# indrajeetadityaroy9/vit-inductive-bias-distillation

Hardware: AMD Instinct MI355X
Metric: distillation images/sec (BASD loss fwd+bwd+grad all-reduce), DeiT-S<-ResNet-50 @ bs256/GPU (higher is better)
Workload: dtype f32; 1 GPU; cfg2 DeiT-S<-ResNet-50 224x224; per_gpu_batch=256, global_batch=256, input_dtype=float32, layout=strided (CLS-sliced / channel-major views), backward=True, grad_allreduce_bytes=88202672, grad_allreduce=none at world size 1 (bucket packed, nothing to exchange), rank_readback=auto, readback_deferred_steps=1756, selector=basd_selector_chain mode 0, parallelism=dp1

## Files before the change

include/basd_hip.h:

```cpp
#ifndef BASD_HIP_H
#define BASD_HIP_H

#include <stdint.h>

#ifdef __cplusplus
extern "C" {
#endif

#ifndef __HIP_PLATFORM_AMD__
typedef struct ihipStream_t* hipStream_t;
#endif

#define BASD_OK 0
#define BASD_EINVAL (-1)
#define BASD_EUNSUPPORTED (-2)
#define BASD_DTYPE_F32 0
#define BASD_DTYPE_BF16 1
#define BASD_DTYPE_U8 2


int basd_gemm_nt(const void* a, int a_dtype, long a_sb, long a_sn, long a_sd, int a_rows_per_batch,
                 long a_batch_stride, const float* b, long ldb, long b_batch_stride, int M, int N, int K, int batch,
                 float* c, long ldc, long c_batch_stride, float scale, const float* bias, float beta,
                 float* colsum_part, float* col_mean, hipStream_t stream);
// ... 134 lines not shown
int basd_selector_chain_tail(const BasdSelectorChain* args, int kmax, int exact_k);
int basd_jacobi_lds_square_fits(int n);


int basd_token_weights(const void* const* attn_ptrs, int dtype, const float* mix, int L, long sb, long sh, long sq,
                       long sk, int B, int H, int A, int has_cls, int n_a, int n_t, int n_s, const int* atap0,
                       const int* atap1, const float* alam, const int* tap0, const int* tap1, const float* lam,
                       float* omega, float* omega_t, float* raw_out, hipStream_t stream);

int basd_student_project(const void* x, int dtype, long sb, long sn, int B, int n_s, int n_t, int D,
                         const float* omega, const int* tap0, const int* tap1, const float* lam, const int* range0,
                         const int* range1, float* mu, float* tr_s, float* a_prime, hipStream_t stream);

int basd_teacher_center(const void* const* tok_ptrs, int dtype, const float* mix, int L, long sb, long sn, long sd,
                        int B, int n, int D, const int* g0, const int* g1, const float* glam, const float* omega_t,
                        float* mu, float* tc, hipStream_t stream);
int basd_teacher_center_multi(const void* const* tok_ptrs, int dtype, const float* mix, int L, int G, long sb, long sn,
                              long sd, int B, int n, int D, const int* g0, const int* g1, const float* glam,
                              const float* omega_t, float* mu, float* tc, hipStream_t stream);
long basd_teacher_center_stream_scratch_floats(int G, int B, int n, int D);
int basd_teacher_center_stream(const void* const* tok_ptrs, int dtype, const float* mix, int L, int G, long sb, long sn,
                               long sd, int B, int n, int D, const int* g0, const int* g1, const float* glam,
                               const float* omega_t, float* mu, float* tc, float* scratch, hipStream_t stream);

int basd_gram_f64(const float* p, long p_batch_stride, int n, int D, int batch, double* g, long g_batch_stride,
                  hipStream_t stream);

int basd_gram_f64_split(const float* p, long p_batch_stride, int n, int D, int batch, int splits, double* slabs,
                        double* g, hipStream_t stream);

int basd_chol_f64(const double* g, long g_batch_stride, int n, int batch, double* l, long l_batch_stride,
                  hipStream_t stream);

int basd_stack_product(const double* la, const double* lb, long l_batch_stride, int n, int batch, int lb_period,
                       float* w, long w_batch_stride, hipStream_t stream);

int basd_procrustes_finalize(const float* w, long w_batch_stride, const float* sigma, int n, int n_s, int batch,
                             int t_period ,
                             const double* gb, long g_batch_stride, const float* omega, const int* tap0,
                             const int* tap1, const float* lam, const float* tr_s_part, int tr_slabs, float* tr_s,
                             float* tr_t, float* nuc, float* loss, float* k_prime, hipStream_t stream);

int basd_student_project_multi(const void* const* x_ptrs, int dtype, long sb, long sn, int E, int B, int n_s, int n_t,
                               int D, int ptrs_16B_aligned, const float* omega, long omega_e_stride, const int* tap0,
                               const int* tap1, const float* lam, const int* range0, const int* range1, float* mu,
                               float* tr_s, float* a_prime, hipStream_t stream);
int basd_student_grad_multi(const void* const* x_ptrs, int dtype, long sb, long sn, int E, int B, int n_s, int n_t,
                            int D, const float* omega, long omega_e_stride, const float* mu, const float* h,
                            const int* tap0, const int* tap1, const float* lam, const float* scale_ptr,
                            float scale_const, float* dx, const float* tnorm2, float* gomega, hipStream_t stream);
int basd_student_grad_fused(const void* const* x_ptrs, int dtype, long sb, long sn, int E, int B, int n_s, int n_t,
                            int D, int ptrs_16B_aligned, const float* omega, long omega_e_stride, const float* mu,
                            const float* k_prime, const float* a_prime, const int* tap0, const int* tap1,
                            const float* lam, const float* scale_ptr, float scale_const, float* dx,
                            hipStream_t stream);

typedef struct BasdProcrustesArgs {
    const void* const* student_ptrs;
    const void* const* student_host_ptrs;
    long s_dtype, s_sb, s_sn, s_aligned;
    const void* const* tok_ptrs;
    long t_dtype, t_sb, t_sn, t_sd;
    const void* const* attn_ptrs;
    long a_dtype, a_sb, a_sh, a_sq, a_sk;
    const float* mix;
    long E, L, G, B, n_s, n_t, d_s, d_t, H, A, has_cls, n_a, n, max_sweeps;
// ... 137 lines not shown
```

vit-inductive-bias-distillation_amd/basd_amd/_lib.py:

```python
from __future__ import annotations

import ctypes as C
import os
import threading

_HERE = os.path.dirname(os.path.abspath(__file__))
LIB_PATH = os.path.join(_HERE, "libbasd_hip.so")

vp, i32, i64, f32, f64 = C.c_void_p, C.c_int, C.c_long, C.c_float, C.c_double

SIGNATURES = {
    "basd_gemm_nt": [vp, i32, i64, i64, i64, i32, i64, vp, i64, i64, i32, i32, i32, i32, vp, i64, i64, f32, vp, f32,
                     vp, vp, vp],
    "basd_gemm_tn_splits": [i32],
    "basd_gemm_tn": [vp, vp, i32, i64, i64, i64, i64, i64, i64, i64, i64, i32, i32, i32, i32, i32, vp, vp, i32, vp,
                     vp, i64, i64, f32, vp],
    "basd_colmean_parts": [i32],
    "basd_colmean": [vp, i32, i64, i64, i64, i32, i64, i32, i32, i32, i32, vp, vp, vp],
    "basd_colmean_multi": [vp, i32, i64, i64, i64, i32, i32, i32, i32, i32, vp, vp, i32, vp],
    "basd_syrk_splits": [i32, i32, i32],
    "basd_syrk_multi": [vp, i32, i64, i64, i64, i32, i32, i32, i32, vp, vp, i32, vp, vp, i64, i32, vp, i32, i32, vp],
    "basd_jacobi_workspace_ints": [i32, i32],
    "basd_jacobi_twopass_workspace_bytes": [i32, i32, i32],
    "basd_jacobi_stacked_twopass": [vp, i64, i32, i32, vp, i32, i32, f32, vp, vp, vp],
# ... 6 lines not shown
    "basd_tridiag_workspace_bytes": [i32, i32],
    "basd_tridiag_tuning": [i32, i32, i32, i32, i32, i32],
    "basd_tridiag": [vp, i64, i32, i32, vp, vp, vp, vp, vp, vp],
    "basd_tridiag_ranked": [vp, i64, i32, i32, vp, vp, vp, vp, vp, i32, f64, i32, vp, vp, vp, vp],
    "basd_tridiag_ranked_gated": [vp, i64, i32, i32, vp, vp, vp, vp, vp, i32, f64, i32, vp, vp, vp, C.c_uint, i32, vp],
    "basd_flag_set": [vp, C.c_uint, vp],
    "basd_scale_unless_one": [vp, i64, vp, vp, vp],
    "basd_event_create": [vp],
    "basd_event_destroy": [vp],
    "basd_stream_wait_event": [vp, vp],
    "basd_tridiag_eigenvalues": [vp, vp, i32, i32, vp, vp],
    "basd_tridiag_apply_q": [vp, vp, i32, i32, i32, vp, vp, i32, i32, vp],
    "basd_tridiag_shifted_solve": [vp, vp, vp, i32, i32, i32, i32, vp, vp, vp],
    "basd_tridiag_mp_rank": [vp, vp, i32, i32, f64, i32, vp, vp, vp, vp, vp],
    "basd_tridiag_mp_rank_rank1": [vp, vp, vp, i32, i32, f64, f64, i32, vp, vp, vp, vp],
    "basd_tridiag_eigenvectors": [vp, vp, vp, vp, vp, i32, i32, i32, vp, vp, i32, vp],
    "basd_mp_rank": [vp, i32, i32, f64, i32, vp, vp, vp],
    "basd_grassmann_distance": [vp, i32, vp, vp, i32, vp, i32, vp, vp, vp],
    "basd_grassmann_distance_padded": [vp, i32, i32, vp, vp, i32, vp, i32, vp, vp],
    "basd_selector_tail": [vp] * 10 + [i32, i32, i32, i32] + [vp] * 14 + [vp],
    "basd_sqrt_clamp": [vp, vp, i64, vp],
    "basd_gram_finish": [vp, vp, i32, i32, i64, vp, vp, vp],
    "basd_cross_entropy": [vp, i32, i64, i32, i32, vp, vp, i64, f32, i64, vp, vp, vp],
    "basd_token_weights": [vp, i32, vp, i32, i64, i64, i64, i64, i32, i32, i32, i32, i32, i32, i32, vp, vp, vp, vp,
                           vp, vp, vp, vp, vp, vp],
    "basd_student_project": [vp, i32, i64, i64, i32, i32, i32, i32, vp, vp, vp, vp, vp, vp, vp, vp, vp, vp],
    "basd_teacher_center": [vp, i32, vp, i32, i64, i64, i64, i32, i32, i32, vp, vp, vp, vp, vp, vp, vp],
    "basd_teacher_center_multi": [vp, i32, vp, i32, i32, i64, i64, i64, i32, i32, i32, vp, vp, vp, vp, vp, vp, vp],
    "basd_teacher_center_stream_scratch_floats": [i32, i32, i32, i32],
    "basd_teacher_center_stream": [vp, i32, vp, i32, i32, i64, i64, i64, i32, i32, i32, vp, vp, vp, vp, vp, vp, vp, vp],
    "basd_gram_f64": [vp, i64, i32, i32, i32, vp, i64, vp],
    "basd_gram_f64_split": [vp, i64, i32, i32, i32, i32, vp, vp, vp],
    "basd_chol_f64": [vp, i64, i32, i32, vp, i64, vp],
    "basd_stack_product": [vp, vp, i64, i32, i32, i32, vp, i64, vp],
    "basd_procrustes_finalize": [vp, i64, vp, i32, i32, i32, i32, vp, i64, vp, vp, vp, vp, vp, i32, vp, vp, vp, vp,
                                 vp, vp],
    "basd_student_project_multi": [vp, i32, i64, i64, i32, i32, i32, i32, i32, i32, vp, i64, vp, vp, vp, vp, vp, vp,
                                   vp, vp, vp],
    "basd_student_grad_multi": [vp, i32, i64, i64, i32, i32, i32, i32, i32, vp, i64, vp, vp, vp, vp, vp, vp, f32, vp,
                                vp, vp, vp],
    "basd_student_grad_fused": [vp, i32, i64, i64, i32, i32, i32, i32, i32, i32, vp, i64, vp, vp, vp, vp, vp, vp, vp,
                                f32, vp, vp],
    "basd_procrustes_forward_fused": [vp, vp],
    "basd_procrustes_tuning": [i32],
    "basd_jacobi_plain4_fits": [i32],
    "basd_stack_product_t": [vp, vp, i64, i32, i32, i32, vp, i64, vp],
    "basd_kprime_from_transposed": [vp, i64, vp, i32, i32, vp, i64, i32, vp, i64, vp, vp],
    "basd_ustack_stash": [vp, i64, i32, i32, vp, i64, vp],
    "basd_ustack_from_transposed": [vp, i64, vp, i32, i32, vp, i64, vp, i64, vp, i32, vp, vp],
    "basd_resample_tokens": [vp, i32, i64, i64, i64, i32, i32, i32, i32, vp, vp, vp, vp, vp],
    "basd_resample_tokens_adjoint": [vp, i32, i32, i32, i32, vp, vp, vp, vp, vp, vp, vp],
    "basd_teacher_factor": [vp, i64, vp, i32, i32, i32, vp, vp, i64, vp, vp, vp, vp, vp, vp, vp, vp, vp],
    "basd_teacher_factor_tiled": [vp, i64, vp, i32, i32, i32, vp, vp, i64, vp, vp, vp, vp, vp, vp, vp, vp, vp, vp],
    "basd_mix_grad_tokens": [vp, vp, i32, i32, i64, i64, i64, i32, i32, i32, i32, vp, vp, vp, vp, vp],
    "basd_mix_grad_tokens_scratch_floats": [i32, i32, i32, i32],
    "basd_mix_grad_tokens_onepass": [vp, vp, i32, i32, i64, i64, i64, i32, i32, i32, i32, vp, vp, vp, vp, vp, vp],
    "basd_token_weight_bwd": [vp, vp, i32, i32, i32, i32, vp, vp, vp, vp, vp, vp, i32, i32, i64, i64, i64, i64, i32,
                              i32, i32, vp, vp, vp],
    "basd_build_angle_stack": [vp, i32, vp, i32, vp, vp],
    "basd_grassmann_distance_bwd": [vp, vp, i32, vp, vp, i32, vp, vp, i32, vp, vp],
    "basd_eigvec_k2": [vp, vp, i32, i32, i32, vp, vp],
    "basd_selector_chain": [vp],
    "basd_rank_certificate": [vp, vp, i32, i32, f64, vp, vp, vp],
    "basd_rank_certificate_scratch_bytes": [i32],
    "basd_debug_fill_lds": [C.c_uint, vp],
    "basd_selector_chain_tail": [vp, i32, i32],
# ... 107 lines not shown
```

vit-inductive-bias-distillation_amd/basd_amd/ops.py:

```python
from __future__ import annotations

from dataclasses import dataclass
from functools import lru_cache

import torch

from . import _lib

import os

F32, BF16 = 0, 1
MAX_SWEEPS = 20
TWO_PASS_SVD = True
TRANSPOSED_MIX_GRAD = True
TWO_PASS_LOG_LIMIT = 16 << 30
EIG_SOLVER = os.environ.get("BASD_EIG_SOLVER", "tridiag")
if os.environ.get("BASD_GEMM_SPLIT") in ("0", "1"):
    _lib.call("basd_gemm_tuning", int(os.environ["BASD_GEMM_SPLIT"]))
if os.environ.get("BASD_JACOBI_ORDERING") in ("0", "1"):
    _lib.call("basd_jacobi_ordering", int(os.environ["BASD_JACOBI_ORDERING"]))


def _stream() -> int:
    return torch._C._cuda_getCurrentRawStream(torch._C._cuda_getDevice())
# ... 475 lines not shown
    if any(o.stride() != out[0].stride() for o in out):
        out = [o.contiguous() for o in out]
    return out


class _ProcrustesPlan:

    def __init__(self, E, L, B, n_s, d_s, n_t, d_t, H, A, has_cls, need_bwd, need_mix_grad, want_sweeps, want_dx,
                 want_uw, dev):
        import ctypes
        self.E, self.L, self.B, self.n_s, self.d_s, self.n_t, self.d_t = E, L, B, n_s, d_s, n_t, d_t
        n_a = A - (1 if has_cls else 0)
        n = min(n_s, n_t)
        self.n, self.n_a = n, n_a
        self.tp = taps(n_t, n_s, dev) if n_t < n_s else None
        self.gt = taps(n_t, n_s, dev) if n_t > n_s else None
        self.atp = taps(n_a, n_s, dev)
        G = self.G = 1 if L == 1 else E
        f32 = dict(device=dev, dtype=torch.float32)
        slabs = (d_s + 31) // 32
        EB, GB = E * B, G * B
        self.need_bwd, self.need_mix_grad, self.want_dx, self.want_uw = need_bwd, need_mix_grad, want_dx, want_uw
        self.kept_sizes = [G * B * n_s, E * B * d_s, EB * n * d_s, EB * n * n if need_bwd else 0, 4 * EB,
                           (4 + 2 * E) if want_uw else 0]
        self.kept_padded = [(c + 63) // 64 * 64 for c in self.kept_sizes]
        self.kept_total = sum(self.kept_padded)
        g_splits = 1
        if GB < 1024 and d_t >= 512:
            g_splits = max(1, min(1024 // GB, d_t // 256, 16))
        self.g_splits = g_splits
        self.g_all = torch.empty((EB + GB + (g_splits * GB if g_splits > 1 else 0), n, n), device=dev, dtype=torch.float64)
        self.l_all = torch.empty((EB + GB, n, n), device=dev, dtype=torch.float64)
        self.W = torch.empty((EB, n, 2 * n), **f32)
        self.tc = torch.empty((G, B, n, d_t), **f32)
        sizes = [GB * n, GB * d_t, EB * slabs, EB * n]
        padded = [(c + 63) // 64 * 64 for c in sizes]
        self.omega_t, self.mu_t, self.tr_part, self.sigma = (
            piece[:c] for piece, c in zip(torch.split(torch.empty((sum(padded),), **f32), padded), sizes))
        self.ints = torch.empty((_lib.query("basd_jacobi_workspace_ints", EB, MAX_SWEEPS) + EB,), device=dev,
                                dtype=torch.int32)
        self.sweeps = self.ints[-EB:] if want_sweeps else None
        transposed_mix = bool(need_mix_grad and need_bwd and _lib.query("basd_jacobi_plain4_fits", n)
                              and (EB >= 128 or TRANSPOSED_MIX_GRAD == "force") and TRANSPOSED_MIX_GRAD)
        jac_bytes = _lib.query("basd_jacobi_twopass_workspace_bytes", n, EB, MAX_SWEEPS) \
            if TWO_PASS_SVD and not transposed_mix else 0
        if jac_bytes > TWO_PASS_LOG_LIMIT or (jac_bytes > (256 << 20)
                                              and jac_bytes > torch.cuda.mem_get_info(dev)[0] // 2):
            jac_bytes = 0
        self.jac_ws = torch.empty((jac_bytes // 8 + 1,), device=dev, dtype=torch.int64) if jac_bytes > 0 else None
        self.h = torch.empty((E, B, n, d_s), **f32) if want_dx else None
        self.w_stack = None
        self.sigma_u = None
        if transposed_mix:
            self.w_stack = torch.empty((EB, n, 2 * n), **f32)
            self.sigma_u = torch.empty((EB, n), **f32)
        self.host_ptrs = (ctypes.c_void_p * E)()

        a = self.args = _lib.ProcrustesArgs()
        a.student_host_ptrs = ctypes.cast(self.host_ptrs, ctypes.c_void_p)
        (a.E, a.L, a.G, a.B, a.n_s, a.n_t, a.d_s, a.d_t, a.H, a.A, a.has_cls, a.n_a, a.n, a.max_sweeps) = \
            E, L, G, B, n_s, n_t, d_s, d_t, H, A, int(has_cls), n_a, n, MAX_SWEEPS
        if self.atp:
            a.atap0, a.atap1, a.alam = self.atp.tap0.data_ptr(), self.atp.tap1.data_ptr(), self.atp.lam.data_ptr()
        if self.tp:
            a.tap0, a.tap1, a.lam = self.tp.tap0.data_ptr(), self.tp.tap1.data_ptr(), self.tp.lam.data_ptr()
            a.range0, a.range1 = self.tp.range0.data_ptr(), self.tp.range1.data_ptr()
        if self.gt:
            a.g0, a.g1, a.glam = self.gt.tap0.data_ptr(), self.gt.tap1.data_ptr(), self.gt.lam.data_ptr()
        a.omega_t, a.mu_t, a.tc, a.tr_part = (self.omega_t.data_ptr(), self.mu_t.data_ptr(), self.tc.data_ptr(),
                                              self.tr_part.data_ptr())
        a.g_all, a.l_all, a.W = self.g_all.data_ptr(), self.l_all.data_ptr(), self.W.data_ptr()
        a.sigma, a.jflags, a.sweeps = self.sigma.data_ptr(), self.ints.data_ptr(), _ptr(self.sweeps)
        a.h = _ptr(self.h)
        a.g_slabs = self.g_all[EB + GB:].data_ptr() if g_splits > 1 else None
        a.g_splits = g_splits
        a.jac_ws = _ptr(self.jac_ws)
        a.w_stack = _ptr(self.w_stack)
        a.sigma_u = _ptr(self.sigma_u)


_PROCRUSTES_PLANS: dict = {}


def procrustes_forward(students: list[torch.Tensor], teachers: list[torch.Tensor], attns: list[torch.Tensor],
                       mix: torch.Tensor, has_cls: bool, *, need_backward: bool = True,
                       want_sweeps: bool = False, need_mix_grad: bool = False,
                       grad_layers: torch.Tensor | None = None,
                       uwso_ce: torch.Tensor | None = None) -> ProcrustesContext:
    import ctypes
    E, L = len(students), len(teachers)
    students = [as_supported(s) for s in students]
    students = _check_common_layout([s if s.stride(2) == 1 else s.contiguous() for s in students],
                                    "student token tensors")
    teachers = _check_common_layout([as_supported(t) for t in teachers], "teacher token tensors")
    attns = _check_common_layout([as_supported(a) for a in attns], "teacher attention tensors")
    _require_cuda(*students, *teachers, *attns, mix)
    s0, t0, a0 = students[0], teachers[0], attns[0]
    dev = s0.device
    B, n_s, d_s = s0.shape
    _, n_t, d_t = t0.shape
    H, A = a0.shape[1], a0.shape[2]
    need_bwd = need_backward or grad_layers is not None
# ... 190 lines not shown
```

vit-inductive-bias-distillation_amd/csrc/fused.hip:

```cpp
#include "basd_common.h"
#include "../../include/basd_hip.h"

namespace basd {

__global__ void __launch_bounds__(256) uwso_combine_kernel(const float* __restrict__ ce, const float* __restrict__ loss_b,
                                                           int E, int B, float* __restrict__ out) {
    constexpr int CH = 32;
    __shared__ double red[CH][4];
    const int tid = threadIdx.x;
    double geo_sum = 0.;
    for (int e0 = 0; e0 < E; e0 += CH) {
        const int ne = E - e0 < CH ? E - e0 : CH;
        for (int e = 0; e < ne; ++e) {
            double acc = 0.;
            for (int b = tid; b < B; b += 256) acc += (double)loss_b[(long)(e0 + e) * B + b];
            for (int m = 32; m > 0; m >>= 1) acc += __shfl_xor(acc, m, 64);
            if ((tid & 63) == 0) red[e][tid >> 6] = acc;
        }
        __syncthreads();
        if (tid == 0)
            for (int e = 0; e < ne; ++e) {
                const float layer = (float)(((red[e][0] + red[e][1]) + (red[e][2] + red[e][3])) / (double)B);
                out[4 + E + e0 + e] = layer;
                geo_sum += (double)layer;
// ... 62 lines not shown
        BASD_TRY(basd_student_grad_multi(a->student_ptrs, (int)a->s_dtype, a->s_sb, a->s_sn, E, B, n_s, n, d_s, a->omega,
                                         om_stride, a->mu_s, a->h, a->tap0, a->tap1, a->lam, grad_layers,
                                         2.0f / (float)B, a->dx, nullptr, nullptr, st));
    }
#undef BASD_TRY
    return BASD_OK;
}

static int g_transposed_cores = 1;
int basd_procrustes_tuning(int transposed_cores) {
    if (transposed_cores >= 0) g_transposed_cores = transposed_cores > 2 ? 2 : transposed_cores;
    return BASD_OK;
}

int basd_procrustes_forward_fused(const BasdProcrustesArgs* a, hipStream_t st) {
    BASD_CHECK_ARG(a && a->student_ptrs && a->tok_ptrs && a->attn_ptrs && a->mix);
    const int E = (int)a->E, L = (int)a->L, G = (int)a->G, B = (int)a->B, n_s = (int)a->n_s, n_t = (int)a->n_t;
    const int d_s = (int)a->d_s, d_t = (int)a->d_t, H = (int)a->H, A = (int)a->A, n_a = (int)a->n_a, n = (int)a->n;
    const float* grad_layers_in = a->grad_layers;
    BASD_CHECK_ARG(E > 0 && L > 0 && (G == 1 || G == E) && B > 0 && n == (n_s < n_t ? n_s : n_t));
    int rc;
#define BASD_TRY(call)            \
    do {                          \
        rc = (call);              \
        if (rc != BASD_OK) return rc; \
    } while (0)
    int centred = BASD_EUNSUPPORTED;
    for (int g = 0; g < G; ++g) {
        BASD_TRY(basd_token_weights(a->attn_ptrs, (int)a->a_dtype, a->mix + (long)g * L, L, a->a_sb, a->a_sh, a->a_sq,
                                    a->a_sk, B, H, A, (int)a->has_cls, n_a, n, n_s, a->atap0, a->atap1, a->alam,
                                    a->tap0, a->tap1, a->lam, a->omega + (long)g * B * n_s,
                                    a->omega_t + (long)g * B * n, a->raw ? a->raw + (long)g * B * n_a : nullptr, st));
    }
    if (G > 1 && L >= 4 && basd_teacher_center_stream_scratch_floats(G, B, n, d_t) <= (long)E * B * 2 * n * n) {
        centred = basd_teacher_center_stream(a->tok_ptrs, (int)a->t_dtype, a->mix, L, G, a->t_sb, a->t_sn, a->t_sd, B, n,
                                             d_t, a->g0, a->g1, a->glam, a->omega_t, a->mu_t, a->tc, a->W, st);
        if (centred != BASD_OK && centred != BASD_EUNSUPPORTED) return centred;
    }
    if (G > 1 && centred != BASD_OK) {
        centred = basd_teacher_center_multi(a->tok_ptrs, (int)a->t_dtype, a->mix, L, G, a->t_sb, a->t_sn, a->t_sd, B, n,
                                            d_t, a->g0, a->g1, a->glam, a->omega_t, a->mu_t, a->tc, st);
        if (centred != BASD_OK && centred != BASD_EUNSUPPORTED) return centred;
    }
    for (int g = 0; g < G && centred != BASD_OK; ++g) {
        BASD_TRY(basd_teacher_center(a->tok_ptrs, (int)a->t_dtype, a->mix + (long)g * L, L, a->t_sb, a->t_sn, a->t_sd,
                                     B, n, d_t, a->g0, a->g1, a->glam, a->omega_t + (long)g * B * n,
                                     a->mu_t + (long)g * B * d_t, a->tc + (long)g * B * n * d_t, st));
    }
    const long om_stride = G == 1 ? 0 : (long)B * n_s;
    int slabs = (d_s + 31) / 32;
    rc = basd_student_project_multi(a->student_ptrs, (int)a->s_dtype, a->s_sb, a->s_sn, E, B, n_s, n, d_s,
                                    (int)a->s_aligned, a->omega, om_stride, a->tap0, a->tap1, a->lam, a->range0,
                                    a->range1, a->mu_s, a->tr_part, a->a_prime, st);
    if (rc == BASD_EUNSUPPORTED) {
        slabs = (d_s + 63) / 64;
        for (int e = 0; e < E; ++e)
            BASD_TRY(basd_student_project(a->student_host_ptrs[e], (int)a->s_dtype, a->s_sb, a->s_sn, B, n_s, n, d_s,
                                          a->omega + e * om_stride, a->tap0, a->tap1, a->lam, a->range0, a->range1,
                                          a->mu_s + (long)e * B * d_s, a->tr_part + (long)e * B * slabs,
                                          a->a_prime + (long)e * B * n * d_s, st));
    } else if (rc != BASD_OK) {
        return rc;
    }
    const long nn = (long)n * n;
    const int EB = E * B, GB = G * B;
    BASD_TRY(basd_gram_f64(a->a_prime, (long)n * d_s, n, d_s, EB, a->g_all, nn, st));
    if (a->g_slabs && a->g_splits > 1)
        BASD_TRY(basd_gram_f64_split(a->tc, (long)n * d_t, n, d_t, GB, (int)a->g_splits, a->g_slabs,
                                     a->g_all + (long)EB * nn, st));
    else
        BASD_TRY(basd_gram_f64(a->tc, (long)n * d_t, n, d_t, GB, a->g_all + (long)EB * nn, nn, st));
    BASD_TRY(basd_chol_f64(a->g_all, nn, n, EB + GB, a->l_all, nn, st));
    if ((a->raw == nullptr || a->w_stack != nullptr) && EB <= 65535 && basd_jacobi_plain4_fits(n) &&
        (g_transposed_cores == 2 || (g_transposed_cores == 1 && EB >= 128))) {
        BASD_TRY(basd_stack_product_t(a->l_all, a->l_all + (long)EB * nn, nn, n, EB, GB, a->W, 2 * nn, st));
        if (a->raw != nullptr) BASD_TRY(basd_ustack_stash(a->W, 2 * nn, n, EB, a->w_stack, 2 * nn, st));
        BASD_TRY(basd_jacobi_onesided(a->W, 2 * nn, n, n, n, EB, nullptr, a->sigma, n, (int)a->max_sweeps, 0.f,
                                      a->jflags, a->sweeps, st));
        BASD_TRY(basd_procrustes_finalize(a->W, 2 * nn, a->sigma, n, n_s, EB, GB, a->g_all + (long)EB * nn, nn, a->omega,
                                          a->tap0, a->tap1, a->lam, a->tr_part, slabs, a->tr_s, a->tr_t, a->nuc,
                                          a->loss_b, nullptr, st));
        if (a->k_prime)
            BASD_TRY(basd_kprime_from_transposed(a->W, 2 * nn, a->sigma, n, EB, a->l_all + (long)EB * nn, nn, GB,
                                                 a->W + nn, 2 * nn, a->k_prime, st));
        if (a->raw != nullptr) {
            BASD_CHECK_ARG(a->sigma_u != nullptr);
            BASD_TRY(basd_ustack_from_transposed(a->W, 2 * nn, a->sigma, n, EB, a->w_stack, 2 * nn, a->W + nn, 2 * nn,
                                                 a->sigma_u, (int)a->max_sweeps, a->jflags, st));
        }
        return procrustes_tail(a, grad_layers_in, E, B, n_s, n, d_s, EB, nn, om_stride, st);
    }
    BASD_TRY(basd_stack_product(a->l_all, a->l_all + (long)EB * nn, nn, n, EB, GB, a->W, 2 * nn, st));
    rc = BASD_EUNSUPPORTED;
    if (a->jac_ws)
        rc = basd_jacobi_stacked_twopass(a->W, 2 * nn, n, EB, a->sigma, n, (int)a->max_sweeps, 0.f, a->jac_ws, a->sweeps,
                                         st);
    if (rc == BASD_EUNSUPPORTED)
        rc = basd_jacobi_onesided(a->W, 2 * nn, n, 2 * n, n, EB, nullptr, a->sigma, n, (int)a->max_sweeps, 0.f,
                                  a->jflags, a->sweeps, st);
    if (rc != BASD_OK) return rc;
    BASD_TRY(basd_procrustes_finalize(a->W, 2 * nn, a->sigma, n, n_s, EB, GB, a->g_all + (long)EB * nn, nn, a->omega,
                                      a->tap0, a->tap1, a->lam, a->tr_part, slabs, a->tr_s, a->tr_t, a->nuc,
                                      a->loss_b, a->k_prime, st));
// ... 22 lines not shown
```

vit-inductive-bias-distillation_amd/csrc/procrustes.hip:

```cpp
#include "basd_common.h"
#include "../../include/basd_hip.h"

namespace basd {

typedef double f64x4 __attribute__((ext_vector_type(4)));

template <typename T>
__global__ void __launch_bounds__(256) token_weights_kernel(const void* const* __restrict__ attn_ptrs,
                                                            const float* __restrict__ mix, int L, long sb, long sh,
                                                            long sq, long sk, int H, int A, int has_cls, int n_a,
                                                            int n_t, int n_s, const int* __restrict__ atap0,
                                                            const int* __restrict__ atap1,
                                                            const float* __restrict__ alam,
                                                            const int* __restrict__ tap0,
                                                            const int* __restrict__ tap1,
                                                            const float* __restrict__ lam, float* __restrict__ omega,
                                                            float* __restrict__ omega_t, float* __restrict__ raw_out) {
    extern __shared__ float sm[];
    float* raw = sm;
    float* w = sm + n_a;
    __shared__ float red[32];
    const int b = blockIdx.x, tid = threadIdx.x;
    for (int j = tid; j < n_a; j += blockDim.x) {
        float acc = 0.f;
// ... 531 lines not shown
                Gb[(long)col * n + row] = acc[t][r];
            }
        }
    }
}

__global__ void __launch_bounds__(256) gram_f64_reduce_kernel(const double* __restrict__ slabs, long split_stride,
                                                              int splits, long count, double* __restrict__ G) {
    const long i = (long)blockIdx.x * 256 + threadIdx.x;
    if (i >= count) return;
    double acc = 0.;
    for (int s2 = 0; s2 < splits; ++s2) acc += slabs[(long)s2 * split_stride + i];
    G[i] = acc;
}

static bool gram_f64_shape(int n, int* waves, int* chunks, size_t* lds) {
    const int nt = (n + 15) / 16, ntiles = nt * (nt + 1) / 2;
    int w = (ntiles + G64_TPW - 1) / G64_TPW;
    if (w < 4) w = ntiles < 4 ? ntiles : 4;
    int c = 1;
    if (w > 16) {
        c = (ntiles + 16 * G64_TPW - 1) / (16 * G64_TPW);
        w = 16;
    }
    *waves = w;
    *chunks = c;
    *lds = sizeof(float) * (size_t)nt * 16 * G64_LD;
    if (*lds > 156 * 1024) return false;
    if (*lds > 48 * 1024)
        (void)hipFuncSetAttribute((const void*)gram_f64_kernel, hipFuncAttributeMaxDynamicSharedMemorySize, 156 * 1024);
    return true;
}

__device__ __forceinline__ int pk(int i, int j, int n) { return j * n - (j * (j - 1)) / 2 + (i - j); }

__global__ void __launch_bounds__(1024) chol_f64_kernel(const double* __restrict__ G, long g_batch_stride, int n,
                                                        double* __restrict__ Lout, long l_batch_stride) {
    extern __shared__ __attribute__((aligned(16))) double a[];
    double* col = a + (size_t)n * (n + 1) / 2;
    __shared__ double sh_piv;
    __shared__ double red[32];
    const int m = blockIdx.x, tid = threadIdx.x, nthr = blockDim.x, lane = tid & 63, wave = tid >> 6, nw = nthr >> 6;
    const double* Gm = G + (long)m * g_batch_stride;
    double dmax = 0.;
    for (int j = wave; j < n; j += nw)
        for (int i = j + lane; i < n; i += 64) {
            const double v = Gm[(long)i * n + j];
            a[pk(i, j, n)] = v;
            if (i == j) dmax = fmax(dmax, v);
        }
    for (int s = 32; s > 0; s >>= 1) dmax = fmax(dmax, __shfl_xor(dmax, s, 64));
    if (lane == 0) red[wave] = dmax;
    __syncthreads();
    dmax = 0.;
    for (int i = 0; i < nw; ++i) dmax = fmax(dmax, red[i]);
    const double thr = dmax * (double)n * 1e-15;
    for (int j = 0; j < n; ++j) {
        if (tid == 0) {
            const double d = a[pk(j, j, n)];
            sh_piv = d > thr ? sqrt(d) : 0.;
        }
        __syncthreads();
        const double piv = sh_piv;
        const double inv = piv > 0. ? 1. / piv : 0.;
        for (int i = j + tid; i < n; i += nthr) {
            const double v = (i == j) ? piv : a[pk(i, j, n)] * inv;
// ... 956 lines not shown
    if (dtype == BASD_DTYPE_F32) LAUNCH_SGF_T(float);
    else if (dtype == BASD_DTYPE_BF16) LAUNCH_SGF_T(__hip_bfloat16);
    else return BASD_EINVAL;
#undef LAUNCH_SGF_T
#undef LAUNCH_SGF
    BASD_RETURN_LAST();
}

int basd_student_project_multi(const void* const* x_ptrs, int dtype, long sb, long sn, int E, int B, int n_s, int n_t,
                               int D, int ptrs_16B_aligned, const float* omega, long omega_e_stride, const int* tap0,
                               const int* tap1, const float* lam, const int* range0, const int* range1, float* mu,
                               float* tr_s, float* a_prime, hipStream_t stream) {
    BASD_CHECK_ARG(x_ptrs && omega && mu && tr_s && a_prime && E > 0 && B > 0 && n_s > 0 && n_t > 0 && D > 0);
    BASD_CHECK_ARG((n_t == n_s) == (tap0 == nullptr));
    BASD_CHECK_ARG(E <= 65535 && B <= 65535);
    const int esz = dtype == BASD_DTYPE_F32 ? 4 : 2;
    const size_t lds = sizeof(float) * ((size_t)n_s * SP_W + 5 * (size_t)n_s);
    const bool ok = ptrs_16B_aligned && D % 4 == 0 && (sb * esz) % 16 == 0 && (sn * esz) % 16 == 0 &&
                    (esz == 4 || D % 8 == 0) && lds <= 96 * 1024;
    if (!ok) return BASD_EUNSUPPORTED;
    const dim3 grid((D + SP_W - 1) / SP_W, B, E);
    if (dtype == BASD_DTYPE_F32) {
        (void)hipFuncSetAttribute((const void*)student_project_v4_kernel<float>, hipFuncAttributeMaxDynamicSharedMemorySize, (int)lds);
        student_project_v4_kernel<float><<<grid, 256, lds, stream>>>(x_ptrs, sb, sn, n_s, n_t, D, omega, omega_e_stride, tap0, tap1, lam, range0, range1, mu, tr_s, a_prime);
    } else if (dtype == BASD_DTYPE_BF16) {
        (void)hipFuncSetAttribute((const void*)student_project_v4_kernel<__hip_bfloat16>, hipFuncAttributeMaxDynamicSharedMemorySize, (int)lds);
        student_project_v4_kernel<__hip_bfloat16><<<grid, 256, lds, stream>>>(x_ptrs, sb, sn, n_s, n_t, D, omega, omega_e_stride, tap0, tap1, lam, range0, range1, mu, tr_s, a_prime);
    } else {
        return BASD_EINVAL;
    }
    BASD_RETURN_LAST();
}

int basd_resample_tokens(const void* x, int dtype, long sb, long sn, long sd, int B, int n_in, int n_out, int D,
                         const int* tap0, const int* tap1, const float* lam, float* out, hipStream_t stream) {
    BASD_CHECK_ARG(x && tap0 && tap1 && lam && out && B > 0 && n_in > 0 && n_out > 0 && D > 0);
    const dim3 grid(n_out, B);
    if (dtype == BASD_DTYPE_F32)
        resample_tokens_kernel<float><<<grid, 128, 0, stream>>>((const float*)x, sb, sn, sd, n_in, n_out, D, tap0, tap1, lam, out);
    else if (dtype == BASD_DTYPE_BF16)
        resample_tokens_kernel<__hip_bfloat16><<<grid, 128, 0, stream>>>((const __hip_bfloat16*)x, sb, sn, sd, n_in, n_out, D, tap0, tap1, lam, out);
    else
        return BASD_EINVAL;
    BASD_RETURN_LAST();
}

int basd_resample_tokens_adjoint(const float* dy, int B, int n_in, int n_out, int D, const int* tap0,
                                 const int* tap1, const float* lam, const int* range0, const int* range1, float* dx,
                                 hipStream_t stream) {
    BASD_CHECK_ARG(dy && tap0 && tap1 && lam && range0 && range1 && dx && B > 0 && n_in > 0 && n_out > 0 && D > 0);
    resample_tokens_adjoint_kernel<<<dim3(n_in, B), 128, 0, stream>>>(dy, n_in, n_out, D, tap0, tap1, lam, range0, range1, dx);
    BASD_RETURN_LAST();
}

}
```

Baseline: 165,100 images/s.

## Fuse Gram f64 accumulation into teacher centering and student projection kernels

Adds two kernels that compute the f64 Gram matrix with MFMA inside the teacher-centering and student-projection passes, working on LDS tiles as they are produced. This removes the separate basd_gram_f64 launches and their re-read of the centred teacher tensor and projected student activations. When no mix gradient is needed, the teacher's centred tensor is no longer allocated or written. In exchange the student kernel now runs one block per (batch, E) instead of splitting D across blocks, which lowers parallelism, and LDS use goes up.

After: 156,500 images/s. 0.948x the previous value.

```diff
diff --git a/include/basd_hip.h b/include/basd_hip.h
--- a/include/basd_hip.h
+++ b/include/basd_hip.h
@@ -190,6 +190,17 @@
 int basd_chol_f64(const double* g, long g_batch_stride, int n, int batch, double* l, long l_batch_stride,
                   hipStream_t stream);
 
+int basd_teacher_center_gram_fits(int n, int gathered);
+int basd_teacher_center_gram(const void* const* tok_ptrs, int dtype, const float* mix, int L, long sb, long sn, long sd,
+                             int B, int n, int D, const int* g0, const int* g1, const float* glam,
+                             const float* omega_t, float* mu, float* tc, int splits, double* slabs, double* g,
+                             hipStream_t stream);
+int basd_student_project_gram_multi(const void* const* x_ptrs, int dtype, long sb, long sn, int E, int B, int n_s,
+                                    int n_t, int D, int ptrs_16B_aligned, const float* omega, long omega_e_stride,
+                                    const int* tap0, const int* tap1, const float* lam, const int* range0,
+                                    const int* range1, float* mu, float* tr_s, float* a_prime, double* g,
+                                    long g_batch_stride, hipStream_t stream);
+
 int basd_stack_product(const double* la, const double* lb, long l_batch_stride, int n, int batch, int lb_period,
                        float* w, long w_batch_stride, hipStream_t stream);
 
diff --git a/vit-inductive-bias-distillation_amd/basd_amd/_lib.py b/vit-inductive-bias-distillation_amd/basd_amd/_lib.py
--- a/vit-inductive-bias-distillation_amd/basd_amd/_lib.py
+++ b/vit-inductive-bias-distillation_amd/basd_amd/_lib.py
@@ -62,6 +62,11 @@
     "basd_gram_f64": [vp, i64, i32, i32, i32, vp, i64, vp],
     "basd_gram_f64_split": [vp, i64, i32, i32, i32, i32, vp, vp, vp],
     "basd_chol_f64": [vp, i64, i32, i32, vp, i64, vp],
+    "basd_teacher_center_gram_fits": [i32, i32],
+    "basd_teacher_center_gram": [vp, i32, vp, i32, i64, i64, i64, i32, i32, i32, vp, vp, vp, vp, vp, vp, i32, vp, vp,
+                                 vp],
+    "basd_student_project_gram_multi": [vp, i32, i64, i64, i32, i32, i32, i32, i32, i32, vp, i64, vp, vp, vp, vp, vp,
+                                        vp, vp, vp, vp, i64, vp],
     "basd_stack_product": [vp, vp, i64, i32, i32, i32, vp, i64, vp],
     "basd_procrustes_finalize": [vp, i64, vp, i32, i32, i32, i32, vp, i64, vp, vp, vp, vp, vp, i32, vp, vp, vp, vp,
                                  vp, vp],
diff --git a/vit-inductive-bias-distillation_amd/basd_amd/ops.py b/vit-inductive-bias-distillation_amd/basd_amd/ops.py
--- a/vit-inductive-bias-distillation_amd/basd_amd/ops.py
+++ b/vit-inductive-bias-distillation_amd/basd_amd/ops.py
@@ -531,7 +531,8 @@
         self.g_all = torch.empty((EB + GB + (g_splits * GB if g_splits > 1 else 0), n, n), device=dev, dtype=torch.float64)
         self.l_all = torch.empty((EB + GB, n, n), device=dev, dtype=torch.float64)
         self.W = torch.empty((EB, n, 2 * n), **f32)
-        self.tc = torch.empty((G, B, n, d_t), **f32)
+        fused_teacher = G == 1 and bool(_lib.query("basd_teacher_center_gram_fits", n, int(bool(self.gt))))
+        self.tc = torch.empty((G, B, n, d_t), **f32) if need_mix_grad or not fused_teacher else None
         sizes = [GB * n, GB * d_t, EB * slabs, EB * n]
         padded = [(c + 63) // 64 * 64 for c in sizes]
         self.omega_t, self.mu_t, self.tr_part, self.sigma = (
@@ -566,7 +567,7 @@
             a.range0, a.range1 = self.tp.range0.data_ptr(), self.tp.range1.data_ptr()
         if self.gt:
             a.g0, a.g1, a.glam = self.gt.tap0.data_ptr(), self.gt.tap1.data_ptr(), self.gt.lam.data_ptr()
-        a.omega_t, a.mu_t, a.tc, a.tr_part = (self.omega_t.data_ptr(), self.mu_t.data_ptr(), self.tc.data_ptr(),
+        a.omega_t, a.mu_t, a.tc, a.tr_part = (self.omega_t.data_ptr(), self.mu_t.data_ptr(), _ptr(self.tc),
                                               self.tr_part.data_ptr())
         a.g_all, a.l_all, a.W = self.g_all.data_ptr(), self.l_all.data_ptr(), self.W.data_ptr()
         a.sigma, a.jflags, a.sweeps = self.sigma.data_ptr(), self.ints.data_ptr(), _ptr(self.sweeps)
diff --git a/vit-inductive-bias-distillation_amd/csrc/fused.hip b/vit-inductive-bias-distillation_amd/csrc/fused.hip
--- a/vit-inductive-bias-distillation_amd/csrc/fused.hip
+++ b/vit-inductive-bias-distillation_amd/csrc/fused.hip
@@ -118,6 +118,18 @@
                                     a->tap0, a->tap1, a->lam, a->omega + (long)g * B * n_s,
                                     a->omega_t + (long)g * B * n, a->raw ? a->raw + (long)g * B * n_a : nullptr, st));
     }
+    const long nn = (long)n * n;
+    const int EB = E * B, GB = G * B;
+    const int t_splits = a->g_slabs && a->g_splits > 1 ? (int)a->g_splits : 1;
+    bool t_gram = false;
+    if (G == 1) {
+        centred = basd_teacher_center_gram(a->tok_ptrs, (int)a->t_dtype, a->mix, L, a->t_sb, a->t_sn, a->t_sd, B, n, d_t,
+                                           a->g0, a->g1, a->glam, a->omega_t, a->mu_t, a->tc, t_splits, a->g_slabs,
+                                           a->g_all + (long)EB * nn, st);
+        if (centred != BASD_OK && centred != BASD_EUNSUPPORTED) return centred;
+        t_gram = centred == BASD_OK;
+    }
+    BASD_CHECK_ARG(t_gram || a->tc != nullptr);
     if (G > 1 && L >= 4 && basd_teacher_center_stream_scratch_floats(G, B, n, d_t) <= (long)E * B * 2 * n * n) {
         centred = basd_teacher_center_stream(a->tok_ptrs, (int)a->t_dtype, a->mix, L, G, a->t_sb, a->t_sn, a->t_sd, B, n,
                                              d_t, a->g0, a->g1, a->glam, a->omega_t, a->mu_t, a->tc, a->W, st);
@@ -135,7 +147,12 @@
     }
     const long om_stride = G == 1 ? 0 : (long)B * n_s;
     int slabs = (d_s + 31) / 32;
-    rc = basd_student_project_multi(a->student_ptrs, (int)a->s_dtype, a->s_sb, a->s_sn, E, B, n_s, n, d_s,
+    rc = basd_student_project_gram_multi(a->student_ptrs, (int)a->s_dtype, a->s_sb, a->s_sn, E, B, n_s, n, d_s,
+                                         (int)a->s_aligned, a->omega, om_stride, a->tap0, a->tap1, a->lam, a->range0,
+                                         a->range1, a->mu_s, a->tr_part, a->a_prime, a->g_all, nn, st);
+    const bool s_gram = rc == BASD_OK;
+    if (rc == BASD_EUNSUPPORTED)
+        rc = basd_student_project_multi(a->student_ptrs, (int)a->s_dtype, a->s_sb, a->s_sn, E, B, n_s, n, d_s,
                                     (int)a->s_aligned, a->omega, om_stride, a->tap0, a->tap1, a->lam, a->range0,
                                     a->range1, a->mu_s, a->tr_part, a->a_prime, st);
     if (rc == BASD_EUNSUPPORTED) {
@@ -148,13 +165,11 @@
     } else if (rc != BASD_OK) {
         return rc;
     }
-    const long nn = (long)n * n;
-    const int EB = E * B, GB = G * B;
-    BASD_TRY(basd_gram_f64(a->a_prime, (long)n * d_s, n, d_s, EB, a->g_all, nn, st));
-    if (a->g_slabs && a->g_splits > 1)
-        BASD_TRY(basd_gram_f64_split(a->tc, (long)n * d_t, n, d_t, GB, (int)a->g_splits, a->g_slabs,
+    if (!s_gram) BASD_TRY(basd_gram_f64(a->a_prime, (long)n * d_s, n, d_s, EB, a->g_all, nn, st));
+    if (!t_gram && t_splits > 1)
+        BASD_TRY(basd_gram_f64_split(a->tc, (long)n * d_t, n, d_t, GB, t_splits, a->g_slabs,
                                      a->g_all + (long)EB * nn, st));
-    else
+    else if (!t_gram)
         BASD_TRY(basd_gram_f64(a->tc, (long)n * d_t, n, d_t, GB, a->g_all + (long)EB * nn, nn, st));
     BASD_TRY(basd_chol_f64(a->g_all, nn, n, EB + GB, a->l_all, nn, st));
     if ((a->raw == nullptr || a->w_stack != nullptr) && EB <= 65535 && basd_jacobi_plain4_fits(n) &&
diff --git a/vit-inductive-bias-distillation_amd/csrc/procrustes.hip b/vit-inductive-bias-distillation_amd/csrc/procrustes.hip
--- a/vit-inductive-bias-distillation_amd/csrc/procrustes.hip
+++ b/vit-inductive-bias-distillation_amd/csrc/procrustes.hip
@@ -587,6 +587,296 @@
     return true;
 }
 
+constexpr int PG_TPW = 3, PG_ROWS = 64;
+
+__device__ __forceinline__ void pg_tiles_of_wave(int wave, int ntiles, int (&ti)[PG_TPW], int (&tj)[PG_TPW]) {
+#pragma unroll
+    for (int t = 0; t < PG_TPW; ++t) {
+        const int lin = wave + 4 * t;
+        int r = 0;
+        while ((r + 1) * (r + 2) / 2 <= lin) ++r;
+        ti[t] = lin < ntiles ? r : -1;
+        tj[t] = lin < ntiles ? lin - r * (r + 1) / 2 : -1;
+    }
+}
+
+__device__ __forceinline__ void pg_chunk_mfma(const float* tile, const int (&ti)[PG_TPW], const int (&tj)[PG_TPW],
+                                              int lane, f64x4 (&acc)[PG_TPW]) {
+    const int i16 = lane & 15, kq = lane >> 4;
+#pragma unroll 1
+    for (int g = 0; g < G64_BK / 16; ++g) {
+#pragma unroll
+        for (int t = 0; t < PG_TPW; ++t) {
+            if (ti[t] < 0) continue;
+            const float4 a = *(const float4*)(tile + (ti[t] * 16 + i16) * G64_LD + g * 16 + 4 * kq);
+            const float4 bb = *(const float4*)(tile + (tj[t] * 16 + i16) * G64_LD + g * 16 + 4 * kq);
+            acc[t] = __builtin_amdgcn_mfma_f64_16x16x4f64((double)a.x, (double)bb.x, acc[t], 0, 0, 0);
+            acc[t] = __builtin_amdgcn_mfma_f64_16x16x4f64((double)a.y, (double)bb.y, acc[t], 0, 0, 0);
+            acc[t] = __builtin_amdgcn_mfma_f64_16x16x4f64((double)a.z, (double)bb.z, acc[t], 0, 0, 0);
+            acc[t] = __builtin_amdgcn_mfma_f64_16x16x4f64((double)a.w, (double)bb.w, acc[t], 0, 0, 0);
+        }
+    }
+}
+
+__device__ __forceinline__ void pg_store(double* __restrict__ Gb, int n, const int (&ti)[PG_TPW],
+                                         const int (&tj)[PG_TPW], int lane, const f64x4 (&acc)[PG_TPW]) {
+#pragma unroll
+    for (int t = 0; t < PG_TPW; ++t) {
+        if (ti[t] < 0) continue;
+        const int col = tj[t] * 16 + (lane & 15);
+#pragma unroll
+        for (int r = 0; r < 4; ++r) {
+            const int row = ti[t] * 16 + (lane >> 4) + 4 * r;
+            if (row < n && col < n) {
+                Gb[(long)row * n + col] = acc[t][r];
+                Gb[(long)col * n + row] = acc[t][r];
+            }
+        }
+    }
+}
+
+template <typename T>
+__global__ void __launch_bounds__(256) teacher_center_gram_kernel(const void* const* __restrict__ tok_ptrs,
+                                                                  const float* __restrict__ mix, int L, long sb,
+                                                                  long sn, long sd, int n, int D,
+                                                                  const float* __restrict__ omega_t,
+                                                                  float* __restrict__ mu_out, float* __restrict__ Tc,
+                                                                  double* __restrict__ G, long g_split_stride) {
+    __shared__ __attribute__((aligned(16))) float raw[G64_BK * PG_ROWS];
+    __shared__ __attribute__((aligned(16))) float tile[PG_ROWS * G64_LD];
+    __shared__ __attribute__((aligned(16))) float mu[G64_BK];
+    __shared__ float wt[PG_ROWS];
+    const int s = blockIdx.x, S = gridDim.x, b = blockIdx.y, tid = threadIdx.x, lane = tid & 63, wave = tid >> 6;
+    const int nt = (n + 15) / 16, total = G64_BK * n;
+    const bool feat_fast = sd == 1;
+    bool vec = sb % 4 == 0 && (feat_fast ? sn % 4 == 0 : (sn == 1 && sd == n));
+    for (int l = 0; l < L; ++l) vec = vec && ((uintptr_t)tok_ptrs[l] & (4 * sizeof(T) - 1)) == 0;
+    const bool tc_vec = Tc != nullptr && D % 4 == 0 && ((uintptr_t)Tc & 15) == 0;
+    int ti[PG_TPW], tj[PG_TPW];
+    pg_tiles_of_wave(wave, nt * (nt + 1) / 2, ti, tj);
+    f64x4 acc[PG_TPW];
+#pragma unroll
+    for (int t = 0; t < PG_TPW; ++t) acc[t] = f64x4{0., 0., 0., 0.};
+    int j0[2], dd0[2], ddl[2];
+#pragma unroll
+    for (int h = 0; h < 2; ++h) {
+        const int e0 = 4 * (tid + 256 * h);
+        if (feat_fast) {
+            j0[h] = e0 >> 5;
+            dd0[h] = e0 & 31;
+            ddl[h] = dd0[h] + 3;
+        } else {
+            dd0[h] = e0 / n;
+            j0[h] = e0 - dd0[h] * n;
+            ddl[h] = (e0 + 3) / n;
+        }
+    }
+    const long base = (long)b * sb;
+    float4 pv[2];
+    auto fetch = [&](int k0) {
+#pragma unroll
+        for (int h = 0; h < 2; ++h) {
+            float x[4] = {0.f, 0.f, 0.f, 0.f};
+            if (4 * (tid + 256 * h) < total) {
+                if (vec && k0 + ddl[h] < D) {
+                    const long off = base + (long)(k0 + dd0[h]) * sd + (long)j0[h] * sn;
+                    for (int l = 0; l < L; ++l) {
+                        const float m = mix[l];
+                        const float4 t4 = ld4f((const BASD_GLOBAL_AS T*)tok_ptrs[l] + off);
+                        x[0] = fmaf(m, t4.x, x[0]); x[1] = fmaf(m, t4.y, x[1]);
+                        x[2] = fmaf(m, t4.z, x[2]); x[3] = fmaf(m, t4.w, x[3]);
+                    }
+                } else {
+                    int j = j0[h], dd = dd0[h];
+#pragma unroll
+                    for (int i = 0; i < 4; ++i) {
+                        if (k0 + dd < D) {
+                            const long off = base + (long)(k0 + dd) * sd + (long)j * sn;
+                            for (int l = 0; l < L; ++l)
+                                x[i] = fmaf(mix[l], ldg_f32((const BASD_GLOBAL_AS T*)tok_ptrs[l] + off), x[i]);
+                        }
+                        if (feat_fast) ++dd;
+                        else if (++j == n) { j = 0; ++dd; }
+                    }
+                }
+            }
+            pv[h] = make_float4(x[0], x[1], x[2], x[3]);
+        }
+    };
+    for (int j = tid; j < n; j += 256) wt[j] = omega_t[(long)b * n + j];
+    for (int i = tid; i < PG_ROWS * G64_LD; i += 256) tile[i] = 0.f;
+    int k0 = s * G64_BK;
+    if (k0 < D) fetch(k0);
+    for (; k0 < D; k0 += G64_BK * S) {
+#pragma unroll
+        for (int h = 0; h < 2; ++h) {
+            const int e0 = 4 * (tid + 256 * h);
+            if (e0 < total) *(float4*)(raw + e0) = pv[h];
+        }
+        if (k0 + G64_BK * S < D) fetch(k0 + G64_BK * S);
+        __syncthreads();
+        if (tid < G64_BK) {
+            float a = 0.f;
+            if (feat_fast) {
+#pragma unroll 8
+                for (int j = 0; j < n; ++j) a = fmaf(wt[j], raw[j * G64_BK + tid], a);
+            } else {
+#pragma unroll 8
+                for (int j = 0; j < n; ++j) a = fmaf(wt[j], raw[tid * n + j], a);
+            }
+            mu[tid] = a;
+            if (k0 + tid < D) mu_out[(long)b * D + k0 + tid] = a;
+        }
+        __syncthreads();
+        for (int idx = tid; idx < n * (G64_BK / 4); idx += 256) {
+            const int j = idx >> 3, c4 = (idx & 7) * 4;
+            float4 v;
+            if (feat_fast) {
+                v = *(const float4*)(raw + j * G64_BK + c4);
+            } else {
+                v.x = raw[c4 * n + j]; v.y = raw[(c4 + 1) * n + j];
+                v.z = raw[(c4 + 2) * n + j]; v.w = raw[(c4 + 3) * n + j];
+            }
+            const float4 m4 = *(const float4*)(mu + c4);
+            v.x -= m4.x; v.y -= m4.y; v.z -= m4.z; v.w -= m4.w;
+            *(float4*)(tile + j * G64_LD + c4) = v;
+            if (Tc) {
+                const int k = k0 + c4;
+                float* o = Tc + ((long)b * n + j) * D + k;
+                if (tc_vec && k + 3 < D) {
+                    *(float4*)o = v;
+                } else {
+                    if (k < D) o[0] = v.x;
+                    if (k + 1 < D) o[1] = v.y;
+                    if (k + 2 < D) o[2] = v.z;
+                    if (k + 3 < D) o[3] = v.w;
+                }
+            }
+        }
+        __syncthreads();
+        pg_chunk_mfma(tile, ti, tj, lane, acc);
+    }
+    pg_store(G + (long)s * g_split_stride + (long)b * n * n, n, ti, tj, lane, acc);
+}
+
+constexpr int SPG_NR = 7;
+template <typename T, bool PREFETCH>
+__global__ void __launch_bounds__(256, 4) student_project_gram_kernel(
+    const void* const* __restrict__ x_ptrs, long sb, long sn, int n_s, int n_t, int D,
+    const float* __restrict__ omega, long omega_e_stride, const int* __restrict__ tap0, const int* __restrict__ tap1,
+    const float* __restrict__ lam, const int* __restrict__ range0, const int* __restrict__ range1,
+    float* __restrict__ mu_out, float* __restrict__ tr_part, float* __restrict__ Ap, double* __restrict__ G,
+    long g_batch_stride) {
+    extern __shared__ __attribute__((aligned(16))) float sm[];
+    float* xs = sm;
+    float* w = sm + (long)n_s * SP_W;
+    float* c0 = w + n_s;
+    float* c1 = c0 + n_s;
+    int* t0 = (int*)(c1 + n_s);
+    int* t1 = t0 + n_s;
+    float* tile = sm + ((37 * n_s + 3) & ~3);
+    float (*red)[SP_W] = (float (*)[SP_W])tile;
+    __shared__ __attribute__((aligned(16))) float mu[SP_W];
+    __shared__ float scratch[32];
+    const int b = blockIdx.x, e = blockIdx.y, B = gridDim.x, tid = threadIdx.x, lane = tid & 63, wave = tid >> 6;
+    const int fq = tid & 7, rg = tid >> 3, c4 = 4 * fq;
+    const int slabs = (D + SP_W - 1) / SP_W, nt = (n_t + 15) / 16, rows_pad = nt * 16;
+    const BASD_GLOBAL_AS T* Xb = (const BASD_GLOBAL_AS T*)x_ptrs[e] + (long)b * sb;
+    const float* om = omega + (long)e * omega_e_stride + (long)b * n_s;
+    int ti[PG_TPW], tj[PG_TPW];
+    pg_tiles_of_wave(wave, nt * (nt + 1) / 2, ti, tj);
+    f64x4 gacc[PG_TPW];
+#pragma unroll
+    for (int t = 0; t < PG_TPW; ++t) gacc[t] = f64x4{0., 0., 0., 0.};
+    for (int n = tid; n < n_s; n += 256) {
+        const float wn = om[n];
+        w[n] = wn;
+        if (tap0) {
+            const float l1 = lam[n];
+            c0[n] = (1.f - l1) * wn;
+            c1[n] = l1 * wn;
+            t0[n] = tap0[n];
+            t1[n] = tap1[n];
+        }
+    }
+    float4 pv[SPG_NR];
+    auto fetch = [&](int d0) {
+        const bool lv = d0 + c4 < D;
+        const BASD_GLOBAL_AS T* p = Xb + d0 + (long)rg * sn + c4;
+#pragma unroll
+        for (int i = 0; i < SPG_NR; ++i, p += 32 * sn) {
+            pv[i] = make_float4(0.f, 0.f, 0.f, 0.f);
+            if (lv && rg + 32 * i < n_s) pv[i] = ld4f(p);
+        }
+    };
+    if (PREFETCH) fetch(0);
+    for (int sl = 0; sl < slabs; ++sl) {
+        const int d0 = sl * SP_W;
+        const bool live = d0 + c4 < D;
+        __syncthreads();
+        if (PREFETCH) {
+#pragma unroll
+            for (int i = 0; i < SPG_NR; ++i) {
+                const int n = rg + 32 * i;
+                if (n < n_s) *(float4*)(xs + n * SP_W + c4) = pv[i];
+            }
+            if (sl + 1 < slabs) fetch(d0 + SP_W);
+        } else {
+            for (int n = rg; n < n_s; n += 32) {
+                float4 v = make_float4(0.f, 0.f, 0.f, 0.f);
+                if (live) v = ld4f(Xb + d0 + (long)n * sn + c4);
+                *(float4*)(xs + n * SP_W + c4) = v;
+            }
+        }
+        __syncthreads();
+        float4 acc = make_float4(0.f, 0.f, 0.f, 0.f);
+        for (int n = rg; n < n_s; n += 32) {
+            const float4 v = *(const float4*)(xs + n * SP_W + c4);
+            const float wn = w[n];
+            acc.x = fmaf(wn, v.x, acc.x); acc.y = fmaf(wn, v.y, acc.y);
+            acc.z = fmaf(wn, v.z, acc.z); acc.w = fmaf(wn, v.w, acc.w);
+        }
+        *(float4*)(&red[rg][c4]) = acc;
+        __syncthreads();
+        if (tid < SP_W) {
+            float m = 0.f;
+#pragma unroll
+            for (int q = 0; q < 32; ++q) m += red[q][tid];
+            mu[tid] = m;
+            if (d0 + tid < D) mu_out[((long)e * B + b) * D + d0 + tid] = m;
+        }
+        __syncthreads();
+        const float4 m4 = *(const float4*)(mu + c4);
+        float part = 0.f;
+        if (live)
+            for (int n = rg; n < n_s; n += 32) {
+                const float4 v = *(const float4*)(xs + n * SP_W + c4);
+                const float cx = v.x - m4.x, cy = v.y - m4.y, cz = v.z - m4.z, cw = v.w - m4.w;
+                part = fmaf(w[n], fmaf(cx, cx, fmaf(cy, cy, fmaf(cz, cz, cw * cw))), part);
+            }
+        const float tr = block_sum(part, scratch);
+        if (tid == 0) tr_part[((long)e * B + b) * slabs + sl] = tr;
+        float* Ab = Ap + ((long)e * B + b) * n_t * D + d0 + c4;
+        for (int j = rg; j < rows_pad; j += 32) {
+            float4 a = make_float4(0.f, 0.f, 0.f, 0.f);
+            if (live && j < n_t) {
+                const int n0 = range0 ? range0[j] : j, n1 = range1 ? range1[j] : j + 1;
+                for (int n = n0; n < n1; ++n) {
+                    const float cw = tap0 ? (t0[n] == j ? c0[n] : 0.f) + (t1[n] == j ? c1[n] : 0.f) : w[n];
+                    const float4 v = *(const float4*)(xs + n * SP_W + c4);
+                    a.x = fmaf(cw, v.x - m4.x, a.x); a.y = fmaf(cw, v.y - m4.y, a.y);
+                    a.z = fmaf(cw, v.z - m4.z, a.z); a.w = fmaf(cw, v.w - m4.w, a.w);
+                }
+                *(float4*)(Ab + (long)j * D) = a;
+            }
+            *(float4*)(tile + j * G64_LD + c4) = a;
+        }
+        __syncthreads();
+        pg_chunk_mfma(tile, ti, tj, lane, gacc);
+    }
+    pg_store(G + ((long)e * B + b) * g_batch_stride, n_t, ti, tj, lane, gacc);
+}
+
 __device__ __forceinline__ int pk(int i, int j, int n) { return j * n - (j * (j - 1)) / 2 + (i - j); }
 
 __global__ void __launch_bounds__(1024) chol_f64_kernel(const double* __restrict__ G, long g_batch_stride, int n,
@@ -1609,6 +1899,66 @@
     BASD_RETURN_LAST();
 }
 
+int basd_teacher_center_gram_fits(int n, int gathered) { return n > 0 && n <= PG_ROWS && !gathered; }
+
+int basd_teacher_center_gram(const void* const* tok_ptrs, int dtype, const float* mix, int L, long sb, long sn, long sd,
+                             int B, int n, int D, const int* g0, const int* g1, const float* glam,
+                             const float* omega_t, float* mu, float* tc, int splits, double* slabs, double* g,
+                             hipStream_t stream) {
+    BASD_CHECK_ARG(tok_ptrs && mix && omega_t && mu && g && L > 0 && B > 0 && n > 0 && D > 0);
+    BASD_CHECK_ARG((g0 == nullptr) == (g1 == nullptr) && (g0 == nullptr) == (glam == nullptr));
+    BASD_CHECK_ARG(splits >= 1 && splits <= 64 && (splits == 1 || slabs != nullptr) && B <= 65535);
+    if (!basd_teacher_center_gram_fits(n, g0 != nullptr)) return BASD_EUNSUPPORTED;
+    const long count = (long)B * n * n;
+    double* out = splits > 1 ? slabs : g;
+    const dim3 grid(splits, B);
+    if (dtype == BASD_DTYPE_F32)
+        teacher_center_gram_kernel<float><<<grid, 256, 0, stream>>>(tok_ptrs, mix, L, sb, sn, sd, n, D, omega_t, mu, tc, out, count);
+    else if (dtype == BASD_DTYPE_BF16)
+        teacher_center_gram_kernel<__hip_bfloat16><<<grid, 256, 0, stream>>>(tok_ptrs, mix, L, sb, sn, sd, n, D, omega_t, mu, tc, out, count);
+    else
+        return BASD_EINVAL;
+    if (splits > 1)
+        gram_f64_reduce_kernel<<<(unsigned)((count + 255) / 256), 256, 0, stream>>>(slabs, count, splits, count, g);
+    BASD_RETURN_LAST();
+}
+
+int basd_student_project_gram_multi(const void* const* x_ptrs, int dtype, long sb, long sn, int E, int B, int n_s,
+                                    int n_t, int D, int ptrs_16B_aligned, const float* omega, long omega_e_stride,
+                                    const int* tap0, const int* tap1, const float* lam, const int* range0,
+                                    const int* range1, float* mu, float* tr_s, float* a_prime, double* g,
+                                    long g_batch_stride, hipStream_t stream) {
+    BASD_CHECK_ARG(x_ptrs && omega && mu && tr_s && a_prime && g && E > 0 && B > 0 && n_s > 0 && n_t > 0 && D > 0);
+    BASD_CHECK_ARG((n_t == n_s) == (tap0 == nullptr));
+    BASD_CHECK_ARG(E <= 65535 && B <= 65535 && ((uintptr_t)a_prime & 15) == 0);
+    if (n_t > PG_ROWS) return BASD_EUNSUPPORTED;
+    const int esz = dtype == BASD_DTYPE_F32 ? 4 : 2;
+    const int rows_pad = (n_t + 15) / 16 * 16, tile_floats = rows_pad * G64_LD > 32 * SP_W ? rows_pad * G64_LD : 32 * SP_W;
+    const size_t lds = sizeof(float) * ((size_t)((37 * n_s + 3) & ~3) + tile_floats);
+    const bool ok = ptrs_16B_aligned && D % 4 == 0 && (sb * esz) % 16 == 0 && (sn * esz) % 16 == 0 &&
+                    (esz == 4 || D % 8 == 0) && lds <= 96 * 1024;
+    if (!ok) return BASD_EUNSUPPORTED;
+    const dim3 grid(B, E);
+#define LAUNCH_SPG(TY, PF)                                                                                            \
+    do {                                                                                                              \
+        (void)hipFuncSetAttribute((const void*)student_project_gram_kernel<TY, PF>,                                   \
+                                  hipFuncAttributeMaxDynamicSharedMemorySize, (int)lds);                              \
+        student_project_gram_kernel<TY, PF><<<grid, 256, lds, stream>>>(x_ptrs, sb, sn, n_s, n_t, D, omega,            \
+                                                                        omega_e_stride, tap0, tap1, lam, range0,      \
+                                                                        range1, mu, tr_s, a_prime, g, g_batch_stride); \
+    } while (0)
+    const bool pf = n_s <= 32 * SPG_NR;
+    if (dtype == BASD_DTYPE_F32) {
+        if (pf) LAUNCH_SPG(float, true); else LAUNCH_SPG(float, false);
+    } else if (dtype == BASD_DTYPE_BF16) {
+        if (pf) LAUNCH_SPG(__hip_bfloat16, true); else LAUNCH_SPG(__hip_bfloat16, false);
+    } else {
+        return BASD_EINVAL;
+    }
+#undef LAUNCH_SPG
+    BASD_RETURN_LAST();
+}
+
 int basd_resample_tokens(const void* x, int dtype, long sb, long sn, long sd, int B, int n_in, int n_out, int D,
                          const int* tap0, const int* tap1, const float* lam, float* out, hipStream_t stream) {
     BASD_CHECK_ARG(x && tap0 && tap1 && lam && out && B > 0 && n_in > 0 && n_out > 0 && D > 0);
```
